# MycroftAI/mycroft-precise

Hardware: NVIDIA H100
Metric: stream-updates/s (16 kHz int16 PCM, 1024-sample chunk -> decoded confidence + trigger) (higher is better)
Workload: dtype f32

## Files before the change

### mycroft_precise_b200/csrc/api.cu

```cuda
#include <cuda_runtime.h>
#include <math.h>
#include <stdarg.h>
#include <stdint.h>
#include <stdio.h>
#include <string.h>

#include <algorithm>
#include <map>
#include <cuda_fp16.h>
#include <limits>
#include <memory>
#include <mutex>
#include <new>
#include <string>
#include <utility>
#include <vector>

#include "../../include/precise_b200.h"
#include "gru_kernels.cuh"
#include "gru_bank.cuh"
#include "gru_wide.cuh"
#include "mfcc_kernels.cuh"
#include "mfcc_fast.cuh"
#include "mfcc_ragged.cuh"
#include "mfcc_tc.cuh"
#include "mfcc_tc3.cuh"
#include "mfcc_mma.cuh"
#include "trigger.cuh"
#include "stream_state.cuh"
#include "history.cuh"
#include "corpus.cuh"
#include "corpus_pool.cuh"
#include "corpus_pairs.cuh"
#include "dataset.cuh"
#include "pool.cuh"
#include "train.cuh"
#include "noise.cuh"

#include <cub/device/device_segmented_sort.cuh>

using namespace pb;

static thread_local char g_err[512] = "";

static int fail(int code, const char* fmt, ...) {
    va_list ap;
    va_start(ap, fmt);
    vsnprintf(g_err, sizeof(g_err), fmt, ap);
    va_end(ap);
    return code;
}

#define CK(call)                                                                                  \
    do {                                                                                          \
        cudaError_t e_ = (call);                                                                  \
        if (e_ != cudaSuccess)                                                                    \
            return fail(PB_ERR_CUDA, "%s failed: %s (%s:%d)", #call, cudaGetErrorString(e_), __FILE__, __LINE__); \
    } while (0)

constexpr int N_PROFILE_SLOTS = 4;
constexpr int PROFILE_POOL = 2048;
constexpr int K2_WARP_PATH_MAX = 8192;
constexpr int64_t HOST_ZERO_COPY_MAX = 64;
constexpr int HOST_PIPE = 3;
constexpr int64_t HOST_SUB_BATCH = 16384;

struct ProfSlot {
    std::vector<cudaEvent_t> ev;
    int used = 0;
    double ms = 0.0;
    uint64_t launches = 0;
};

template <typename T>
class DevArray {
public:
    DevArray() = default;
    DevArray(DevArray&& o) noexcept : p_(o.p_), n_(o.n_) { o.p_ = nullptr; o.n_ = 0; }
    DevArray& operator=(DevArray&& o) noexcept { std::swap(p_, o.p_); std::swap(n_, o.n_); return *this; }
    DevArray(const DevArray&) = delete;
    DevArray& operator=(const DevArray&) = delete;
    ~DevArray() { if (p_) cudaFree(p_); }

    cudaError_t alloc(size_t n) {
        T* p = nullptr;
        const cudaError_t e = cudaMalloc((void**)&p, std::max<size_t>(n, 1) * sizeof(T));
        if (e != cudaSuccess) return e;
        DevArray fresh;
        fresh.p_ = p; fresh.n_ = n;
        *this = std::move(fresh);
        return cudaSuccess;
    }
    cudaError_t upload(const std::vector<T>& v) {
        DevArray fresh;
        cudaError_t e = fresh.alloc(v.size());
        if (e == cudaSuccess && !v.empty()) e = cudaMemcpy(fresh.p_, v.data(), v.size() * sizeof(T), cudaMemcpyHostToDevice);
        if (e == cudaSuccess) *this = std::move(fresh);
        return e;
    }
    T* get() const { return p_; }
    size_t size() const { return n_; }

private:
    T* p_ = nullptr;
    size_t n_ = 0;
};

struct NetWeights {
    bool small_path = false;
    GruSmallW<20, 13> w_small;
    DevArray<float> wcat, bias, wd;
    float bd = 0.f;
    DevArray<uint4> bfrag16;
    DevArray<uint4> xfrag16;
    DevArray<float> mma_bias, mma_wd;
    bool wide_ok = false;
    int wg_fp = 0, wg_hp = 0;
    DevArray<uint4> wg_b1, wg_b2; DevArray<float> wg_bias;
};

struct StreamTrig {
    double sensitivity;
    int32_t trigger_level;
    int32_t chunk_bytes;
};

struct Network {
    pb_config cfg;
    std::vector<double> cd;
    int min_out = 0, max_out = 0;
    DevArray<double> d_cd;
    DevArray<int> trig;
    int gru_mode = 0;
    std::unique_ptr<NetWeights> w;
    bool trig_set = false;
    std::vector<StreamTrig> trig_host;
    DevArray<TrigRec> trig_rec;
};

struct pb_handle {
    pb_config cfg;
    int sm_count = 132;
    int used = 0, n_bins = 0, n_out = 0, feat = 0, ring_rows = 0, row_stride = 0, tail_cap = 0, max_new = 0;
    int rel_window = 0;
    size_t k1_batch_smem = 0, k1_stream_smem = 0, k1_fast_smem = 0, k1_pipe_smem = 0, k1_ragged_smem = 0;
    bool ragged = false;
    bool force_generic = false;
    int k1_mode = 0;
    bool mma_ok = false;
    DevArray<uint2> d_mm_b1, d_mm_b2; DevArray<float2> d_mm_tw;
    DevArray<MmRec> d_mm_recs; DevArray<unsigned int> d_mm_counters;
    int mm_parity = 0;
    bool fast_ok = false;
    int npl = 0, maxc = 0, nol = 0;
    DevArray<float4> d_ptab;
    DevArray<unsigned char> d_ctab;
    DevArray<float> d_dct_t;
    bool pipe_fixed = false;
    DevArray<int4> d_pm_off; DevArray<float4> d_pm_w; DevArray<uint4> d_pm_crow; DevArray<float4> d_pm_dct;
    std::vector<double> fb;
    DevArray<float> d_wrise, d_wfall, d_dct;
    DevArray<int> d_grid;
    DevArray<float2> d_tw_stage, d_tw_post, d_tw_any;
    DevArray<long long> d_n_samples;
    DevArray<int16_t> d_tail;
    DevArray<float> d_ring;
    std::vector<Network> models;
    bool routed = false;
    std::vector<uint8_t> route_mask;
    int64_t subs[PB_MAX_MODELS] = {};
    DevArray<uint8_t> d_route;
    DevArray<int2> d_route_list;
    DevArray<unsigned> d_route_count;
// ... 719 lines not shown
                    power257[k] = (k == 0 || k == 256) ? re * re * inv : (re * re + im * im) * inv;
                }
    }
    return PB_OK;
}

PB_API int pb_debug_mma_dft_power(const int16_t* x512, double* power257) {
    if (!x512 || !power257) return fail(PB_ERR_INVALID, "null argument");
    mm_host_power(x512, power257);
    return PB_OK;
}

PB_API int pb_debug_force_generic(pb_handle* h, int on) { if (!h) return fail(PB_ERR_INVALID, "null handle"); h->force_generic = on != 0; return PB_OK; }

PB_API int pb_profile_enable(pb_handle* h, int on) { if (!h) return fail(PB_ERR_INVALID, "null handle"); h->profiling = on != 0; return PB_OK; }

PB_API int pb_profile_reset(pb_handle* h) {
    if (!h) return fail(PB_ERR_INVALID, "null handle");
    for (auto& p : h->prof) { p.used = 0; p.ms = 0; p.launches = 0; }
    return PB_OK;
}

PB_API int pb_profile_read(pb_handle* h, double ms[4], uint64_t launches[4]) {
    if (!h) return fail(PB_ERR_INVALID, "null handle");
    CK(cudaSetDevice(h->cfg.device));
    for (int s = 0; s < N_PROFILE_SLOTS; ++s) {
        ProfSlot& p = h->prof[s];
        for (int i = 0; i + 1 < p.used; i += 2) {
            CK(cudaEventSynchronize(p.ev[i + 1]));
            float t = 0; CK(cudaEventElapsedTime(&t, p.ev[i], p.ev[i + 1])); p.ms += t;
        }
        p.used = 0;
        if (ms) ms[s] = p.ms;
        if (launches) launches[s] = p.launches;
    }
    return PB_OK;
}

static MelTables mel_tables(const pb_handle* h) {
    MelTables t;
    t.w_rise = h->d_wrise.get(); t.w_fall = h->d_wfall.get(); t.grid = h->d_grid.get(); t.dct = h->d_dct.get();
    t.tw_stage = h->d_tw_stage.get(); t.tw_post = h->d_tw_post.get();
    t.n_bins = h->n_bins; t.n_filt = h->cfg.n_filt; t.n_out = h->n_out;
    t.mels_only = h->cfg.vectorizer == PB_VEC_MELS;
    t.n_fft = h->cfg.n_fft; t.tw_any = h->d_tw_any.get();
    return t;
}

static FastTables fast_tables(const pb_handle* h) {
    FastTables f;
    f.ptab = h->d_ptab.get(); f.ctab = h->d_ctab.get(); f.dct_t = h->d_dct_t.get();
    f.npl = h->npl; f.maxc = h->maxc; f.nol = h->nol;
    return f;
}

static StreamState stream_state(const pb_handle* h) {
    StreamState st;
    st.n_samples = h->d_n_samples.get(); st.tail = h->d_tail.get(); st.ring = h->d_ring.get();
    st.tail_cap = h->tail_cap; st.ring_rows = h->ring_rows; st.row_stride = h->row_stride;
    return st;
}

static int trigger_reset(long long bytes) {
    long long q = -(8 * 2048) / bytes;
    if ((-(8 * 2048)) % bytes != 0) q -= 1;
    return (int)q;
}

static DecodeParams decode_params(const Network& net) {
    const pb_config& c = net.cfg;
    DecodeParams d;
    d.cd = net.d_cd.get(); d.cd_len = (int)net.cd.size();
    d.min_out = net.min_out; d.out_range = net.max_out - net.min_out;
    d.center = c.threshold_center;
    d.hot_threshold = 1.0 - c.sensitivity;
    d.trigger_level = c.trigger_level;
    d.trigger_reset = trigger_reset(2LL * c.chunk_samples);
    d.legacy_f64 = c.decode_legacy_f64 != 0;
    return d;
}

static StreamTrig default_trig(const Network& net) {
    return StreamTrig{net.cfg.sensitivity, net.cfg.trigger_level, (int32_t)std::min<long long>(2LL * net.cfg.chunk_samples, INT32_MAX)};
}

static TrigRec trig_record(const StreamTrig& v) {
    return TrigRec{1.0 - v.sensitivity, v.trigger_level, trigger_reset(v.chunk_bytes)};
}

static void defer_trigger(TrigTick& t, int& nt, const Network& net, unsigned route_bit, K2Out& o) {
    t.conf[nt] = o.conf; t.fired[nt] = o.fired; t.count[nt] = o.count; t.trig[nt] = o.trig;
    t.rec[nt] = net.trig_rec.get(); t.route_bit[nt] = route_bit;
    ++nt;
    o.trig = nullptr; o.fired = nullptr; o.count = nullptr;
}

static int launch_trigger(const TrigTick& t, int nt, cudaStream_t s) {
    if (nt == 0 || t.n == 0) return PB_OK;
    trigger_kernel<<<dim3((unsigned)((t.n + 255) / 256), (unsigned)nt), 256, 0, s>>>(t);
    CK(cudaGetLastError());
    return PB_OK;
}

template <typename T>
static int mfcc_impl(pb_handle* h, const T* d_in, int64_t n_streams, int64_t L, float* d_out, cudaStream_t s, float scale) {
    if (!h) return fail(PB_ERR_INVALID, "null handle");
    if (n_streams < 0 || L < 0) return fail(PB_ERR_INVALID, "negative size");
    if (L == 0 && n_streams > 0) return fail(PB_ERR_INVALID, "Cannot vectorize empty audio!");
    const int64_t nf = pb_mfcc_frames(h, L), total = nf * n_streams;
    if (total == 0) return PB_OK;
    if (!d_in || !d_out) return fail(PB_ERR_INVALID, "null buffer");
    CK(cudaSetDevice(h->cfg.device));
    const bool pairs = (L % 2 == 0) && (h->cfg.hop_samples % 2 == 0) && (h->used % 2 == 0) &&
                       ((uintptr_t)d_in % (2 * sizeof(T)) == 0);
    const int64_t tiles = (total + K1_TILE - 1) / K1_TILE;
    const int grid = (int)std::min<int64_t>(tiles, (int64_t)h->sm_count * 4);
    ProfScope ps(h, 0, s);
    if (sizeof(T) == 2 && h->fast_ok && L % 8 == 0 && (uintptr_t)d_in % 16 == 0 && !h->force_generic) {
        const int64_t pairs2 = (total + 1) / 2;
        const int gridf = (int)std::min<int64_t>((pairs2 + K1F_WARPS - 1) / K1F_WARPS, (int64_t)h->sm_count * 4);
        mfcc_fast_batch_kernel<<<gridf, K1F_THREADS, h->k1_fast_smem, s>>>((const int16_t*)d_in, L, nf, total, h->cfg.hop_samples, scale,
                                                                           mel_tables(h), fast_tables(h), d_out);
    } else if (pairs)
        mfcc_batch_kernel<T, true><<<grid, K1_THREADS, h->k1_batch_smem, s>>>(d_in, L, nf, total, h->cfg.hop_samples, h->used, scale, mel_tables(h), d_out);
    else
        mfcc_batch_kernel<T, false><<<grid, K1_THREADS, h->k1_batch_smem, s>>>(d_in, L, nf, total, h->cfg.hop_samples, h->used, scale, mel_tables(h), d_out);
    CK(cudaGetLastError());
    return PB_OK;
}

PB_API int pb_mfcc(pb_handle* h, const int16_t* d_pcm, int64_t n_streams, int64_t L, float* d_out, void* stream) {
    if (!h) return fail(PB_ERR_INVALID, "null handle");
    const float inv = 1.0f / 32768.0f;
    return mfcc_impl<int16_t>(h, d_pcm, n_streams, L, d_out, (cudaStream_t)stream, inv * inv / (float)h->cfg.n_fft);
}

PB_API int pb_mfcc_f32(pb_handle* h, const float* d_audio, int64_t n_streams, int64_t L, float* d_out, void* stream) {
    if (!h) return fail(PB_ERR_INVALID, "null handle");
    return mfcc_impl<float>(h, d_audio, n_streams, L, d_out, (cudaStream_t)stream, 1.0f / (float)h->cfg.n_fft);
}

static void set_bank_slot(BankParams& P, int slot, const Network& net, const K2Out& o) {
    const NetWeights& nw = *net.w;
    BankModelW& w = P.w[slot];
    w.bfrag = nw.bfrag16.get(); w.xfrag = nw.xfrag16.get(); w.bias = nw.mma_bias.get(); w.wd = nw.mma_wd.get(); w.bd = nw.bd;
    w.act = net.cfg.activation; w.ract = net.cfg.recurrent_activation;
    P.dp[slot] = decode_params(net);
    P.o[slot] = o;
}

template <int NM, bool RING, bool KERAS_ACT>
static int launch_bank_act(const BankParams& P, const K2In& in, int64_t n, cudaStream_t s) {
    constexpr size_t smem = (size_t)NM * BANK_MODEL_SMEM + (bank_stages(NM, RING) ? BANK_STAGE_SMEM : 0);
    if constexpr (smem > 48 * 1024) CK(ensure_dyn_smem(gru_bank_kernel<NM, RING, KERAS_ACT>, smem));
    const int per_cta = (MMA_THREADS / 32) * 16;
    gru_bank_kernel<NM, RING, KERAS_ACT><<<(int)((n + per_cta - 1) / per_cta), MMA_THREADS, smem, s>>>(P, in, n);
    CK(cudaGetLastError());
    return PB_OK;
}

template <int NM, bool RING>
static int launch_bank_nm(const BankParams& P, const K2In& in, int64_t n, cudaStream_t s) {
    if constexpr (NM == 1)
        if (P.w[0].act == PB_ACT_LINEAR && P.w[0].ract == PB_RACT_HARD_SIGMOID) return launch_bank_act<1, RING, true>(P, in, n, s);
    return launch_bank_act<NM, RING, false>(P, in, n, s);
}

static int launch_gru_kernels(const Network& net, int F, const K2In& in, bool ring, int64_t n, const K2Out& o, cudaStream_t s) {
    const NetWeights& nw = *net.w;
    const pb_config& c = net.cfg;
    const DecodeParams dp = decode_params(net);
    if (nw.small_path && n <= K2_WARP_PATH_MAX && net.gru_mode == 0) {
        const int grid = (int)((n + 3) / 4);
        if (ring) gru_warp_kernel<20, 13, true><<<grid, 128, 0, s>>>(nw.w_small, in, n, dp, o);
        else gru_warp_kernel<20, 13, false><<<grid, 128, 0, s>>>(nw.w_small, in, n, dp, o);
    } else if (nw.small_path && net.gru_mode != 1) {
        BankParams P{};
        set_bank_slot(P, 0, net, o);
        return ring ? launch_bank_nm<1, true>(P, in, n, s) : launch_bank_nm<1, false>(P, in, n, s);
    } else if (nw.small_path) {
        const int per_cta = K2_SMALL_THREADS * K2_NS;
        const int grid = (int)((n + per_cta - 1) / per_cta);
        if (ring && o.route) gru_small_kernel<20, 13, true, true><<<grid, K2_SMALL_THREADS, 0, s>>>(nw.w_small, in, n, dp, o);
        else if (ring) gru_small_kernel<20, 13, true><<<grid, K2_SMALL_THREADS, 0, s>>>(nw.w_small, in, n, dp, o);
        else gru_small_kernel<20, 13, false><<<grid, K2_SMALL_THREADS, 0, s>>>(nw.w_small, in, n, dp, o);
    } else if (nw.wide_ok && net.gru_mode != 1) {
        GruWideW w;
        w.b1 = nw.wg_b1.get(); w.b2 = nw.wg_b2.get(); w.bias = nw.wg_bias.get(); w.wd = nw.wd.get(); w.bd = nw.bd;
        w.H = c.hidden; w.F = F; w.FP = nw.wg_fp; w.HP = nw.wg_hp; w.act = c.activation; w.ract = c.recurrent_activation;
        const int grid = (int)((n + WG_STREAMS - 1) / WG_STREAMS);
        const size_t smem = wg_smem(w.FP, w.HP);
        if (ring) gru_wide_kernel<true><<<grid, WG_THREADS, smem, s>>>(w, in, n, dp, o);
        else gru_wide_kernel<false><<<grid, WG_THREADS, smem, s>>>(w, in, n, dp, o);
    } else {
        GruTiledW w;
        w.wcat = nw.wcat.get(); w.bias = nw.bias.get(); w.wd = nw.wd.get(); w.bd = nw.bd;
        w.H = c.hidden; w.F_in = F; w.act = c.activation; w.ract = c.recurrent_activation;
        const size_t smem = (size_t)(w.F_in + 3 * w.H) * K2_TILE_STREAMS * sizeof(float);
        const int grid = (int)((n + K2_TILE_STREAMS - 1) / K2_TILE_STREAMS);
        if (ring) gru_tiled_kernel<true><<<grid, K2_TILE_THREADS, smem, s>>>(w, in, n, dp, o);
        else gru_tiled_kernel<false><<<grid, K2_TILE_THREADS, smem, s>>>(w, in, n, dp, o);
    }
    CK(cudaGetLastError());
    return PB_OK;
}

static int launch_gru(pb_handle* h, const Network& net, const K2In& in, bool ring, int64_t n, const K2Out& o, cudaStream_t s) {
    ProfScope ps(h, 1, s);
    return launch_gru_kernels(net, h->feat, in, ring, n, o, s);
}

PB_API int pb_predict(pb_handle* h, const float* d_inputs, int64_t n, float* d_out, float* d_logit, void* stream) {
    if (!h) return fail(PB_ERR_INVALID, "null handle");
    if (!h->models[0].w) return fail(PB_ERR_STATE, "pb_load_weights has not been called");
    if (n < 0) return fail(PB_ERR_INVALID, "negative n");
    if (n == 0) return PB_OK;
    if (!d_inputs || !d_out) return fail(PB_ERR_INVALID, "null buffer");
    CK(cudaSetDevice(h->cfg.device));
    K2In in{};
    in.inputs = d_inputs; in.row_stride = h->feat; in.T = h->cfg.n_features; in.F_base = h->n_out; in.use_delta = 0;
    K2Out o{};
    o.raw = d_out; o.logit = d_logit;
    return launch_gru(h, h->models[0], in, false, n, o, (cudaStream_t)stream);
}

PB_API int pb_decode(pb_handle* h, const float* d_raw, int64_t n, double* d_conf, void* stream) {
    if (!h) return fail(PB_ERR_INVALID, "null handle");
    if (n < 0) return fail(PB_ERR_INVALID, "negative n");
    if (n == 0) return PB_OK;
    if (!d_raw || !d_conf) return fail(PB_ERR_INVALID, "null buffer");
    CK(cudaSetDevice(h->cfg.device));
    cudaStream_t s = (cudaStream_t)stream;
    ProfScope ps(h, 2, s);
    decode_kernel<<<(int)((n + 255) / 256), 256, 0, s>>>(d_raw, n, decode_params(h->models[0]), d_conf);
    CK(cudaGetLastError());
    return PB_OK;
}

static int check_tick(pb_handle* h, const void* pcm, int64_t n) {
    if (!h) return fail(PB_ERR_INVALID, "null handle");
    if (n < 0 || n > h->cfg.max_streams) return fail(PB_ERR_INVALID, "n = %lld outside [0, max_streams = %d]", (long long)n, h->cfg.max_streams);
    if (n > 0 && !pcm) return fail(PB_ERR_INVALID, "null pcm");
    return PB_OK;
}

static int ensure_mma_tables(pb_handle* h) {
    if (h->d_mm_b1.get()) return PB_OK;
    std::vector<uint2> b1, b2;
    std::vector<float2> tw;
    mm_build_tables(b1, b2, tw);
    CK(h->d_mm_b2.upload(b2));
    CK(h->d_mm_tw.upload(tw));
    CK(h->d_mm_recs.alloc((size_t)h->cfg.max_streams * (size_t)std::max(1, h->max_new)));
    CK(h->d_mm_counters.alloc(2));
    CK(cudaMemset(h->d_mm_counters.get(), 0, 2 * sizeof(unsigned int)));
    CK(ensure_dyn_smem(mfcc_mma_kernel<false, false>, sizeof(MmSmem)));
    CK(ensure_dyn_smem(mfcc_mma_kernel<true, false>, sizeof(MmSmem)));
    CK(ensure_dyn_smem(mfcc_mma_kernel<true, true>, sizeof(MmSmem)));
    CK(h->d_mm_b1.upload(b1));
    return PB_OK;
}

static int launch_ragged_mfcc(pb_handle* h, const int16_t* d_pcm, const int64_t* d_offsets, int64_t max_len, const int32_t* d_ids,
                              int64_t n, cudaStream_t s) {
    const float inv = 1.0f / 32768.0f, scale = inv * inv / (float)h->cfg.n_fft;
    const StreamState st = stream_state(h);
    RaggedIn rg;
    rg.offsets = reinterpret_cast<const long long*>(d_offsets);
    rg.max_len = max_len;
    rg.chunk = h->cfg.chunk_samples;
    rg.sub = 6 * h->cfg.hop_samples;
    const bool fast = h->fast_ok && !h->force_generic;
    const int64_t warps_total = (int64_t)h->sm_count * 4 * K1F_WARPS;
    const int spw = (int)std::max<int64_t>(1, std::min<int64_t>(K1F_STREAMS_PER_WARP, (n + warps_total - 1) / warps_total));
    const int64_t tilesf = (n + spw - 1) / spw;
    const int gridf = (int)std::min<int64_t>((tilesf + K1F_WARPS - 1) / K1F_WARPS, (int64_t)h->sm_count * 4);
    const int grid = (int)std::min<int64_t>((n + K1_STREAMS_PER_CTA - 1) / K1_STREAMS_PER_CTA, (int64_t)h->sm_count * 4);
    ProfScope ps(h, 0, s);
    for (int64_t off = 0; off < max_len; off += rg.sub) {
        rg.round_off = off;
        if (fast)
            mfcc_ragged_stream_kernel<<<gridf, K1F_THREADS, h->k1_ragged_smem, s>>>(d_pcm, rg, d_ids, (int)n, h->cfg.hop_samples, spw, scale,
                                                                                   mel_tables(h), fast_tables(h), st);
        else
            mfcc_stream_kernel<false, true><<<grid, K1_THREADS, h->k1_stream_smem, s>>>(d_pcm, d_ids, (int)n, 0, 0, h->cfg.hop_samples, h->used,
                                                                                       scale, mel_tables(h), st, rg);
        CK(cudaGetLastError());
    }
    return PB_OK;
}

static int launch_stream_mfcc(pb_handle* h, const int16_t* d_pcm, const int32_t* d_ids, int64_t n, cudaStream_t s) {
    if (h->ragged) return launch_ragged_mfcc(h, d_pcm, nullptr, h->cfg.chunk_samples, d_ids, n, s);
    const bool pairs = (h->cfg.chunk_samples % 2 == 0) && (h->cfg.hop_samples % 2 == 0) && (h->used % 2 == 0) &&
                       ((uintptr_t)d_pcm % 4 == 0);
    const int64_t tiles = (n + K1_STREAMS_PER_CTA - 1) / K1_STREAMS_PER_CTA;
    const int grid = (int)std::min<int64_t>(tiles, (int64_t)h->sm_count * 4);
    const float inv = 1.0f / 32768.0f, scale = inv * inv / (float)h->cfg.n_fft;
    const StreamState st = stream_state(h);
    ProfScope ps(h, 0, s);
    if (h->k1_mode >= 4 && h->mma_ok && (uintptr_t)d_pcm % 16 == 0 && !h->force_generic) {
        int rc = ensure_mma_tables(h);
        if (rc != PB_OK) return rc;
        MmTables t;
        t.b1 = h->d_mm_b1.get(); t.b2 = h->d_mm_b2.get(); t.tw = h->d_mm_tw.get();
        t.pscale = inv * inv / (float)h->cfg.n_fft * 1024.f;
        const int par = h->mm_parity;
        h->mm_parity ^= 1;
        MmRec* recs = h->d_mm_recs.get();
// ... 2446 lines not shown
```

### mycroft_precise_b200/csrc/gru_bank.cuh

```cuda
#pragma once
#include <cuda_fp16.h>

#include "gru_kernels.cuh"

namespace pb {

__device__ __forceinline__ void mma_f16_k16(float (&d)[4], const uint32_t (&a)[4], uint32_t b0, uint32_t b1) {
    asm volatile("mma.sync.aligned.m16n8k16.row.col.f32.f16.f16.f32 {%0,%1,%2,%3}, {%4,%5,%6,%7}, {%8,%9}, {%0,%1,%2,%3};"
                 : "+f"(d[0]), "+f"(d[1]), "+f"(d[2]), "+f"(d[3])
                 : "r"(a[0]), "r"(a[1]), "r"(a[2]), "r"(a[3]), "r"(b0), "r"(b1));
}
__device__ __forceinline__ void mma_f16_k8(float (&d)[4], uint32_t a0, uint32_t a1, uint32_t b0) {
    asm volatile("mma.sync.aligned.m16n8k8.row.col.f32.f16.f16.f32 {%0,%1,%2,%3}, {%4,%5}, {%6}, {%0,%1,%2,%3};"
                 : "+f"(d[0]), "+f"(d[1]), "+f"(d[2]), "+f"(d[3])
                 : "r"(a0), "r"(a1), "r"(b0));
}
__device__ __forceinline__ uint32_t pack_f16x2_sat(float x, float y) {
    uint32_t r;
    asm("cvt.rn.satfinite.f16x2.f32 %0, %1, %2;" : "=r"(r) : "f"(y), "f"(x));
    return r;
}
__device__ __forceinline__ void split_f16(float x, float y, uint32_t& hi, uint32_t& lo) {
    hi = pack_f16x2_sat(x, y);
    const float2 f = __half22float2(*reinterpret_cast<const __half2*>(&hi));
// ... 105 lines not shown
            idx[hf] = p.x;
            sid[hf] = p.y;
        } else if (RING && ok[hf]) {
            sid[hf] = in.ids ? in.ids[idx[hf]] : (int)idx[hf];
        }
        if (RING && ok[hf]) {
            if (!STAGE) {
                const long long ns = in.n_samples[sid[hf]];
                rc[hf].init(in, sid[hf], ns >= in.window ? (ns - in.window) / in.hop + 1 : 0);
            }
        }
    }
    float* stage = reinterpret_cast<float*>(bank_smem + NM * BANK_MODEL_SMEM) + warp * 2 * BANK_STAGE_BUF;
    const int cs = lane >> 1;
    const bool cok = STAGE && base + cs < n;
    RingCursor cur;
    cur.stride = 0;
    if (cok) {
        const int csid = list != nullptr ? list[base + cs].y : in.ids ? in.ids[base + cs] : (int)(base + cs);
        const long long ns = in.n_samples[csid];
        cur.init(in, csid, ns >= in.window ? (ns - in.window) / in.hop + 1 : 0);
    }
    if (STAGE) {
        bank_stage(stage, cur, cok, cs, 0, in.T, in.ring, lane);
        cp_async_commit();
        bank_stage(stage + BANK_STAGE_BUF, cur, cok, cs, BANK_STAGE_STEPS, in.T, in.ring, lane);
        cp_async_commit();
    }
    int chunk = 0, cr = 0;
    float hreg[NM][3][4];
#pragma unroll
    for (int m = 0; m < NM; ++m)
#pragma unroll
        for (int nt = 0; nt < 3; ++nt)
#pragma unroll
            for (int e = 0; e < 4; ++e) hreg[m][nt][e] = 0.f;

#pragma unroll 1
    for (int step = 0; step < in.T; ++step) {
        float xv[2][4];
        if (STAGE) {
            if (cr == 0) {
                cp_async_wait<1>();
                __syncwarp();
            }
            const float* xs = stage + (chunk & 1) * BANK_STAGE_BUF + cr * 16 * BANK_STAGE_ROW;
#pragma unroll
            for (int hf = 0; hf < 2; ++hf) {
                const float* row = xs + (g + 8 * hf) * BANK_STAGE_ROW;
                const float2 lo = *reinterpret_cast<const float2*>(row + 2 * t), hi = *reinterpret_cast<const float2*>(row + 2 * t + 8);
                xv[hf][0] = 2 * t < F ? lo.x : 0.f;
                xv[hf][1] = 2 * t + 1 < F ? lo.y : 0.f;
                xv[hf][2] = 2 * t + 8 < F ? hi.x : 0.f;
                xv[hf][3] = 2 * t + 9 < F ? hi.y : 0.f;
            }
            if (cr + 1 == BANK_STAGE_STEPS) {
                __syncwarp();
                bank_stage(stage + (chunk & 1) * BANK_STAGE_BUF, cur, cok, cs, (chunk + 2) * BANK_STAGE_STEPS, in.T, in.ring, lane);
                cp_async_commit();
                cr = 0;
                ++chunk;
            } else {
                ++cr;
            }
        } else {
#pragma unroll
            for (int hf = 0; hf < 2; ++hf) {
                const float* row = nullptr;
                if (ok[hf]) row = RING ? rc[hf].next(step) : input_row(in, idx[hf], step);
                xv[hf][0] = (row != nullptr && 2 * t < F) ? __ldg(row + 2 * t) : 0.f;
                xv[hf][1] = (row != nullptr && 2 * t + 1 < F) ? __ldg(row + 2 * t + 1) : 0.f;
                xv[hf][2] = (row != nullptr && 2 * t + 8 < F) ? __ldg(row + 2 * t + 8) : 0.f;
                xv[hf][3] = (row != nullptr && 2 * t + 9 < F) ? __ldg(row + 2 * t + 9) : 0.f;
            }
        }
        uint32_t xh[4], xl[4];
        split_f16(xv[0][0], xv[0][1], xh[0], xl[0]);
        split_f16(xv[1][0], xv[1][1], xh[1], xl[1]);
        split_f16(xv[0][2], xv[0][3], xh[2], xl[2]);
        split_f16(xv[1][2], xv[1][3], xh[3], xl[3]);
#pragma unroll
        for (int m = 0; m < NM; ++m) {
            const uint4* sB = reinterpret_cast<const uint4*>(bank_smem + (ws + m) * BANK_MODEL_SMEM);
            const uint4* sX = sB + 2 * MMA_NT * 32;
            const float* sBias = reinterpret_cast<const float*>(sB + BANK_FRAG_U4);
            const int ra = P.w[m0 + m].ract, ac = P.w[m0 + m].act;
            float acc[MMA_NT][4];
#pragma unroll
            for (int nt = 0; nt < MMA_NT; ++nt) {
                const float b0 = sBias[8 * nt + 2 * t], b1 = sBias[8 * nt + 2 * t + 1];
                acc[nt][0] = b0; acc[nt][1] = b1; acc[nt][2] = b0; acc[nt][3] = b1;
            }
#pragma unroll
            for (int ng = 0; ng < MMA_NT; ng += 3) {
                uint4 w[3];
#pragma unroll
                for (int q = 0; q < 3; ++q) w[q] = sX[(ng + q) * 32 + lane];
#pragma unroll
                for (int q = 0; q < 3; ++q) mma_f16_k16(acc[ng + q], xl, w[q].x, w[q].y);
#pragma unroll
                for (int q = 0; q < 3; ++q) mma_f16_k16(acc[ng + q], xh, w[q].z, w[q].w);
#pragma unroll
                for (int q = 0; q < 3; ++q) mma_f16_k16(acc[ng + q], xh, w[q].x, w[q].y);
            }
            {
                uint32_t ah[4], al[4], ch[2], cl[2];
                frag_f16(hreg[m], ah, al, ch, cl);
                mma3_f16(acc, 0, ah, al, ch, cl, sB, lane);
                mma3_f16(acc, 3, ah, al, ch, cl, sB, lane);
            }
            {
                float rh[3][4];
#pragma unroll
                for (int nt = 0; nt < 3; ++nt)
#pragma unroll
                    for (int e = 0; e < 4; ++e) {
                        const float r = KERAS_ACT ? hard_sigmoid(acc[3 + nt][e]) : apply_ract(acc[3 + nt][e], ra);
                        rh[nt][e] = __fmul_rn(r, hreg[m][nt][e]);
                    }
                uint32_t ah[4], al[4], ch[2], cl[2];
                frag_f16(rh, ah, al, ch, cl);
                mma3_f16(acc, 6, ah, al, ch, cl, sB, lane);
            }
#pragma unroll
            for (int nt = 0; nt < 3; ++nt)
#pragma unroll
                for (int e = 0; e < 4; ++e) {
                    const float z = KERAS_ACT ? hard_sigmoid(acc[nt][e]) : apply_ract(acc[nt][e], ra);
                    const float a = KERAS_ACT ? acc[6 + nt][e] : apply_act(acc[6 + nt][e], ac);
                    hreg[m][nt][e] = __fmaf_rn(z, hreg[m][nt][e], __fmul_rn(__fsub_rn(1.f, z), a));
                }
        }
    }
    if (STAGE) cp_async_wait<0>();
#pragma unroll
    for (int m = 0; m < NM; ++m) {
        const float* sWd = reinterpret_cast<const float*>(bank_smem + (ws + m) * BANK_MODEL_SMEM + BANK_FRAG_U4 * 16) + 72;
#pragma unroll
        for (int hf = 0; hf < 2; ++hf) {
            float part = 0.f;
#pragma unroll
            for (int nt = 0; nt < 3; ++nt) {
                part = fmaf(hreg[m][nt][2 * hf], sWd[8 * nt + 2 * t], part);
                part = fmaf(hreg[m][nt][2 * hf + 1], sWd[8 * nt + 2 * t + 1], part);
            }
            part += __shfl_xor_sync(0xffffffffu, part, 1);
            part += __shfl_xor_sync(0xffffffffu, part, 2);
            epilogue(part + P.w[m0 + m].bd, t == 0 && ok[hf], idx[hf], sid[hf], P.dp[m0 + m], P.o[m0 + m]);
        }
    }
}

template <int NM, bool RING, bool KERAS_ACT>
__global__ void __launch_bounds__(MMA_THREADS, NM == 1 ? 4 : 1)
gru_bank_kernel(const __grid_constant__ BankParams P, K2In in, long long n) {
    bank_scan<NM, RING, KERAS_ACT>(P, 0, nullptr, blockIdx.x, in, n);
}

struct BankRoute {
    const int2* list[BANK_MAX_MODELS];
    const unsigned* count[BANK_MAX_MODELS];
    int tile0[BANK_MAX_MODELS + 1];
    int nm;
};

struct RouteOut {
    float* raw;
    double* conf;
    uint8_t* fired;
    int M;
    int2* lists;
    long long list_stride;
    unsigned* count;
    unsigned listed;
};

__global__ void __launch_bounds__(256) route_kernel(const uint8_t* route, const int* ids, long long n, RouteOut r) {
    const long long i = (long long)blockIdx.x * blockDim.x + threadIdx.x;
    const bool ok = i < n;
    const int sid = ok ? (ids ? ids[i] : (int)i) : 0;
    const unsigned mask = ok ? route[sid] : 0u;
    const int lane = threadIdx.x & 31;
    for (int m = 0; m < r.M; ++m) {
        const unsigned bit = 1u << m;
        const long long o = (long long)m * n + i;
        if (ok && !(mask & bit)) {
            if (r.raw) r.raw[o] = __int_as_float(0x7fc00000);
            r.conf[o] = __longlong_as_double(0x7ff8000000000000LL);
            if (r.fired) r.fired[o] = 0;
        }
        if (r.lists != nullptr && (r.listed & bit)) {
            const bool sub = ok && (mask & bit);
            const unsigned b = __ballot_sync(0xffffffffu, sub);
            if (b == 0) continue;
            unsigned at = 0;
            if (lane == 0) at = atomicAdd(r.count + m, (unsigned)__popc(b));
            at = __shfl_sync(0xffffffffu, at, 0);
            if (sub) r.lists[m * r.list_stride + at + __popc(b & ((1u << lane) - 1u))] = make_int2((int)i, sid);
        }
    }
}

template <bool KERAS_ACT>
__global__ void __launch_bounds__(MMA_THREADS, 4)
gru_bank_routed_kernel(const __grid_constant__ BankParams P, const __grid_constant__ BankRoute R, K2In in) {
    int k = 0;
    while (k + 1 < R.nm && (int)blockIdx.x >= R.tile0[k + 1]) ++k;
    const long long tile = (long long)blockIdx.x - R.tile0[k];
    const long long n = *R.count[k];
    if (tile * (MMA_THREADS / 32) * 16 >= n) return;
    bank_scan<1, true, KERAS_ACT>(P, k, R.list[k], tile, in, n);
}

}
```

Measured before the change: 305.2 million.

## Replace per-warp mma.sync GRU scan with Hopper wgmma kernel for single-model bank

Adds a new GRU scan kernel for the single-model bank path. It stores the split-fp16 weight tiles in shared memory in the wgmma core-matrix layout and issues warpgroup-level wgmma.mma_async (m64n24/48/72) instead of per-warp m16n8k16 mma.sync. The aim is fewer instructions per recurrent step and operand reuse across the warpgroup, at the cost of async fence/commit/wait overhead on every step. The multi-model bank kernel's launch bounds are relaxed to one block per SM, since single-model launches now go to the new kernel.

```diff
diff --git a/mycroft_precise_b200/csrc/api.cu b/mycroft_precise_b200/csrc/api.cu
--- a/mycroft_precise_b200/csrc/api.cu
+++ b/mycroft_precise_b200/csrc/api.cu
@@ -19,6 +19,7 @@
 #include "../../include/precise_b200.h"
 #include "gru_kernels.cuh"
 #include "gru_bank.cuh"
+#include "gru_wg.cuh"
 #include "gru_wide.cuh"
 #include "mfcc_kernels.cuh"
 #include "mfcc_fast.cuh"
@@ -1044,9 +1045,15 @@
 template <int NM, bool RING, bool KERAS_ACT>
 static int launch_bank_act(const BankParams& P, const K2In& in, int64_t n, cudaStream_t s) {
     constexpr size_t smem = (size_t)NM * BANK_MODEL_SMEM + (bank_stages(NM, RING) ? BANK_STAGE_SMEM : 0);
-    if constexpr (smem > 48 * 1024) CK(ensure_dyn_smem(gru_bank_kernel<NM, RING, KERAS_ACT>, smem));
     const int per_cta = (MMA_THREADS / 32) * 16;
-    gru_bank_kernel<NM, RING, KERAS_ACT><<<(int)((n + per_cta - 1) / per_cta), MMA_THREADS, smem, s>>>(P, in, n);
+    const int grid = (int)((n + per_cta - 1) / per_cta);
+    if constexpr (NM == 1) {
+        if constexpr (smem > 48 * 1024) CK(ensure_dyn_smem(gru_wg_kernel<RING, KERAS_ACT>, smem));
+        gru_wg_kernel<RING, KERAS_ACT><<<grid, MMA_THREADS, smem, s>>>(P, in, n);
+    } else {
+        if constexpr (smem > 48 * 1024) CK(ensure_dyn_smem(gru_bank_kernel<NM, RING, KERAS_ACT>, smem));
+        gru_bank_kernel<NM, RING, KERAS_ACT><<<grid, MMA_THREADS, smem, s>>>(P, in, n);
+    }
     CK(cudaGetLastError());
     return PB_OK;
 }
diff --git a/mycroft_precise_b200/csrc/gru_bank.cuh b/mycroft_precise_b200/csrc/gru_bank.cuh
--- a/mycroft_precise_b200/csrc/gru_bank.cuh
+++ b/mycroft_precise_b200/csrc/gru_bank.cuh
@@ -281,7 +281,7 @@
 }
 
 template <int NM, bool RING, bool KERAS_ACT>
-__global__ void __launch_bounds__(MMA_THREADS, NM == 1 ? 4 : 1)
+__global__ void __launch_bounds__(MMA_THREADS, 1)
 gru_bank_kernel(const __grid_constant__ BankParams P, K2In in, long long n) {
     bank_scan<NM, RING, KERAS_ACT>(P, 0, nullptr, blockIdx.x, in, n);
 }
diff --git a/mycroft_precise_b200/csrc/gru_wg.cuh b/mycroft_precise_b200/csrc/gru_wg.cuh
--- /dev/null
+++ b/mycroft_precise_b200/csrc/gru_wg.cuh
@@ -0,0 +1,235 @@
+#pragma once
+#include <stdint.h>
+
+#include "gru_bank.cuh"
+
+namespace pb {
+
+constexpr int WG_TILE_BYTES = 72 * 16 * 2;
+__host__ __device__ constexpr int wg_b_offset(int k, int n) { return (n >> 3) * 256 + (k >> 3) * 128 + (n & 7) * 16 + (k & 7) * 2; }
+
+__device__ __forceinline__ uint64_t wg_desc(const void* p) {
+    const uint32_t a = (uint32_t)__cvta_generic_to_shared(p);
+    return (uint64_t)((a & 0x3ffff) >> 4) | ((uint64_t)(128 >> 4) << 16) | ((uint64_t)(256 >> 4) << 32);
+}
+
+__device__ __forceinline__ void wg_fence() { asm volatile("wgmma.fence.sync.aligned;" ::: "memory"); }
+__device__ __forceinline__ void wg_commit() { asm volatile("wgmma.commit_group.sync.aligned;" ::: "memory"); }
+template <int N>
+__device__ __forceinline__ void wg_wait() { asm volatile("wgmma.wait_group.sync.aligned %0;" :: "n"(N) : "memory"); }
+__device__ __forceinline__ void wg_fence_smem() { asm volatile("fence.proxy.async.shared::cta;" ::: "memory"); }
+template <int N>
+__device__ __forceinline__ void wg_fence_regs(float* d) {
+#pragma unroll
+    for (int i = 0; i < N; ++i) asm volatile("" : "+f"(d[i]) :: "memory");
+}
+
+__device__ __forceinline__ void wgmma_n24(float* d, const uint32_t (&a)[4], uint64_t desc) {
+    asm volatile("{\n.reg .pred p;\nsetp.ne.b32 p, %17, 0;\n"
+                 "wgmma.mma_async.sync.aligned.m64n24k16.f32.f16.f16 "
+                 "{%0,%1,%2,%3,%4,%5,%6,%7,%8,%9,%10,%11}, {%12,%13,%14,%15}, %16, p, 1, 1, 0;\n}\n"
+                 : "+f"(d[0]), "+f"(d[1]), "+f"(d[2]), "+f"(d[3]), "+f"(d[4]), "+f"(d[5]), "+f"(d[6]), "+f"(d[7]),
+                   "+f"(d[8]), "+f"(d[9]), "+f"(d[10]), "+f"(d[11])
+                 : "r"(a[0]), "r"(a[1]), "r"(a[2]), "r"(a[3]), "l"(desc), "r"(1));
+}
+__device__ __forceinline__ void wgmma_n48(float* d, const uint32_t (&a)[4], uint64_t desc) {
+    asm volatile("{\n.reg .pred p;\nsetp.ne.b32 p, %29, 0;\n"
+                 "wgmma.mma_async.sync.aligned.m64n48k16.f32.f16.f16 "
+                 "{%0,%1,%2,%3,%4,%5,%6,%7,%8,%9,%10,%11,%12,%13,%14,%15,%16,%17,%18,%19,%20,%21,%22,%23}, "
+                 "{%24,%25,%26,%27}, %28, p, 1, 1, 0;\n}\n"
+                 : "+f"(d[0]), "+f"(d[1]), "+f"(d[2]), "+f"(d[3]), "+f"(d[4]), "+f"(d[5]), "+f"(d[6]), "+f"(d[7]),
+                   "+f"(d[8]), "+f"(d[9]), "+f"(d[10]), "+f"(d[11]), "+f"(d[12]), "+f"(d[13]), "+f"(d[14]), "+f"(d[15]),
+                   "+f"(d[16]), "+f"(d[17]), "+f"(d[18]), "+f"(d[19]), "+f"(d[20]), "+f"(d[21]), "+f"(d[22]), "+f"(d[23])
+                 : "r"(a[0]), "r"(a[1]), "r"(a[2]), "r"(a[3]), "l"(desc), "r"(1));
+}
+__device__ __forceinline__ void wgmma_n72(float* d, const uint32_t (&a)[4], uint64_t desc) {
+    asm volatile("{\n.reg .pred p;\nsetp.ne.b32 p, %41, 0;\n"
+                 "wgmma.mma_async.sync.aligned.m64n72k16.f32.f16.f16 "
+                 "{%0,%1,%2,%3,%4,%5,%6,%7,%8,%9,%10,%11,%12,%13,%14,%15,%16,%17,%18,%19,%20,%21,%22,%23,"
+                 "%24,%25,%26,%27,%28,%29,%30,%31,%32,%33,%34,%35}, {%36,%37,%38,%39}, %40, p, 1, 1, 0;\n}\n"
+                 : "+f"(d[0]), "+f"(d[1]), "+f"(d[2]), "+f"(d[3]), "+f"(d[4]), "+f"(d[5]), "+f"(d[6]), "+f"(d[7]),
+                   "+f"(d[8]), "+f"(d[9]), "+f"(d[10]), "+f"(d[11]), "+f"(d[12]), "+f"(d[13]), "+f"(d[14]), "+f"(d[15]),
+                   "+f"(d[16]), "+f"(d[17]), "+f"(d[18]), "+f"(d[19]), "+f"(d[20]), "+f"(d[21]), "+f"(d[22]), "+f"(d[23]),
+                   "+f"(d[24]), "+f"(d[25]), "+f"(d[26]), "+f"(d[27]), "+f"(d[28]), "+f"(d[29]), "+f"(d[30]), "+f"(d[31]),
+                   "+f"(d[32]), "+f"(d[33]), "+f"(d[34]), "+f"(d[35])
+                 : "r"(a[0]), "r"(a[1]), "r"(a[2]), "r"(a[3]), "l"(desc), "r"(1));
+}
+
+template <bool RING, bool KERAS_ACT>
+__global__ void __launch_bounds__(MMA_THREADS, 4)
+gru_wg_kernel(const __grid_constant__ BankParams P, K2In in, long long n) {
+    extern __shared__ __align__(16) unsigned char bank_smem[];
+    const BankModelW& w = P.w[0];
+    unsigned char* sW = bank_smem;
+    float* sb = reinterpret_cast<float*>(bank_smem + BANK_FRAG_U4 * 16);
+    for (int e = threadIdx.x; e < 3 * MMA_NT * 32; e += blockDim.x) {
+        const int kt = e / (MMA_NT * 32), nt = (e / 32) % MMA_NT, lane = e & 31, col = 8 * nt + (lane >> 2), k = 2 * (lane & 3);
+        const uint4 f = kt < 2 ? __ldg(w.bfrag + e) : __ldg(w.xfrag + e - 2 * MMA_NT * 32);
+        unsigned char* hi = sW + (kt == 2 ? 0 : 2 + 2 * kt) * WG_TILE_BYTES;
+        unsigned char* lo = hi + WG_TILE_BYTES;
+        *reinterpret_cast<uint32_t*>(hi + wg_b_offset(k, col)) = f.x;
+        *reinterpret_cast<uint32_t*>(hi + wg_b_offset(k + 8, col)) = f.y;
+        *reinterpret_cast<uint32_t*>(lo + wg_b_offset(k, col)) = f.z;
+        *reinterpret_cast<uint32_t*>(lo + wg_b_offset(k + 8, col)) = f.w;
+    }
+    for (int e = threadIdx.x; e < 72; e += blockDim.x) sb[e] = __ldg(w.bias + e);
+    for (int e = threadIdx.x; e < 24; e += blockDim.x) sb[72 + e] = __ldg(w.wd + e);
+    wg_fence_smem();
+    __syncthreads();
+    const int lane = threadIdx.x & 31, warp = threadIdx.x >> 5, g = lane >> 2, t = lane & 3;
+    const long long base = ((long long)blockIdx.x * (MMA_THREADS / 32) + warp) * 16;
+    constexpr bool STAGE = RING;
+    const int F = in.F_base;
+    long long idx[2];
+    int sid[2];
+    bool ok[2];
+#pragma unroll
+    for (int hf = 0; hf < 2; ++hf) {
+        idx[hf] = base + g + 8 * hf;
+        ok[hf] = idx[hf] < n;
+        sid[hf] = RING && ok[hf] ? (in.ids ? in.ids[idx[hf]] : (int)idx[hf]) : 0;
+    }
+    float* stage = reinterpret_cast<float*>(bank_smem + BANK_MODEL_SMEM) + warp * 2 * BANK_STAGE_BUF;
+    const int cs = lane >> 1;
+    const bool cok = STAGE && base + cs < n;
+    RingCursor cur;
+    cur.stride = 0;
+    if (cok) {
+        const int csid = in.ids ? in.ids[base + cs] : (int)(base + cs);
+        const long long ns = in.n_samples[csid];
+        cur.init(in, csid, ns >= in.window ? (ns - in.window) / in.hop + 1 : 0);
+    }
+    if (STAGE) {
+        bank_stage(stage, cur, cok, cs, 0, in.T, in.ring, lane);
+        cp_async_commit();
+        bank_stage(stage + BANK_STAGE_BUF, cur, cok, cs, BANK_STAGE_STEPS, in.T, in.ring, lane);
+        cp_async_commit();
+    }
+    const uint64_t dXh = wg_desc(sW), dXl = wg_desc(sW + WG_TILE_BYTES), dU0h = wg_desc(sW + 2 * WG_TILE_BYTES),
+                   dU0l = wg_desc(sW + 3 * WG_TILE_BYTES), dU1h = wg_desc(sW + 4 * WG_TILE_BYTES), dU1l = wg_desc(sW + 5 * WG_TILE_BYTES);
+    constexpr uint64_t C6 = (6 * 256) >> 4;
+    const int ra = w.ract, ac = w.act;
+    int chunk = 0, cr = 0;
+    float h[3][4] = {};
+
+#pragma unroll 1
+    for (int step = 0; step < in.T; ++step) {
+        float xv[2][4];
+        if (STAGE) {
+            if (cr == 0) {
+                cp_async_wait<1>();
+                __syncwarp();
+            }
+            const float* xs = stage + (chunk & 1) * BANK_STAGE_BUF + cr * 16 * BANK_STAGE_ROW;
+#pragma unroll
+            for (int hf = 0; hf < 2; ++hf) {
+                const float* row = xs + (g + 8 * hf) * BANK_STAGE_ROW;
+                const float2 lo = *reinterpret_cast<const float2*>(row + 2 * t), hi = *reinterpret_cast<const float2*>(row + 2 * t + 8);
+                xv[hf][0] = 2 * t < F ? lo.x : 0.f;
+                xv[hf][1] = 2 * t + 1 < F ? lo.y : 0.f;
+                xv[hf][2] = 2 * t + 8 < F ? hi.x : 0.f;
+                xv[hf][3] = 2 * t + 9 < F ? hi.y : 0.f;
+            }
+            if (cr + 1 == BANK_STAGE_STEPS) {
+                __syncwarp();
+                bank_stage(stage + (chunk & 1) * BANK_STAGE_BUF, cur, cok, cs, (chunk + 2) * BANK_STAGE_STEPS, in.T, in.ring, lane);
+                cp_async_commit();
+                cr = 0;
+                ++chunk;
+            } else {
+                ++cr;
+            }
+        } else {
+#pragma unroll
+            for (int hf = 0; hf < 2; ++hf) {
+                const float* row = ok[hf] ? input_row(in, idx[hf], step) : nullptr;
+                xv[hf][0] = (row != nullptr && 2 * t < F) ? __ldg(row + 2 * t) : 0.f;
+                xv[hf][1] = (row != nullptr && 2 * t + 1 < F) ? __ldg(row + 2 * t + 1) : 0.f;
+                xv[hf][2] = (row != nullptr && 2 * t + 8 < F) ? __ldg(row + 2 * t + 8) : 0.f;
+                xv[hf][3] = (row != nullptr && 2 * t + 9 < F) ? __ldg(row + 2 * t + 9) : 0.f;
+            }
+        }
+        uint32_t xh[4], xl[4];
+        split_f16(xv[0][0], xv[0][1], xh[0], xl[0]);
+        split_f16(xv[1][0], xv[1][1], xh[1], xl[1]);
+        split_f16(xv[0][2], xv[0][3], xh[2], xl[2]);
+        split_f16(xv[1][2], xv[1][3], xh[3], xl[3]);
+        float acc[36];
+#pragma unroll
+        for (int nt = 0; nt < MMA_NT; ++nt) {
+            const float b0 = sb[8 * nt + 2 * t], b1 = sb[8 * nt + 2 * t + 1];
+            acc[4 * nt] = b0; acc[4 * nt + 1] = b1; acc[4 * nt + 2] = b0; acc[4 * nt + 3] = b1;
+        }
+        uint32_t ah[4], al[4], ch[4] = {0u, 0u, 0u, 0u}, cl[4] = {0u, 0u, 0u, 0u};
+        {
+            uint32_t c2h[2], c2l[2];
+            frag_f16(h, ah, al, c2h, c2l);
+            ch[0] = c2h[0]; ch[1] = c2h[1]; cl[0] = c2l[0]; cl[1] = c2l[1];
+        }
+        wg_fence_regs<36>(acc);
+        wg_fence();
+        wgmma_n48(acc, xl, dXh);
+        wgmma_n24(acc + 24, xl, dXh + C6);
+        wgmma_n48(acc, xh, dXl);
+        wgmma_n24(acc + 24, xh, dXl + C6);
+        wgmma_n48(acc, xh, dXh);
+        wgmma_n24(acc + 24, xh, dXh + C6);
+        wgmma_n48(acc, al, dU0h);
+        wgmma_n48(acc, cl, dU1h);
+        wgmma_n48(acc, ah, dU0l);
+        wgmma_n48(acc, ch, dU1l);
+        wgmma_n48(acc, ah, dU0h);
+        wgmma_n48(acc, ch, dU1h);
+        wg_commit();
+        wg_wait<0>();
+        wg_fence_regs<36>(acc);
+        {
+            float rh[3][4];
+#pragma unroll
+            for (int nt = 0; nt < 3; ++nt)
+#pragma unroll
+                for (int e = 0; e < 4; ++e) {
+                    const float r = KERAS_ACT ? hard_sigmoid(acc[4 * (3 + nt) + e]) : apply_ract(acc[4 * (3 + nt) + e], ra);
+                    rh[nt][e] = __fmul_rn(r, h[nt][e]);
+                }
+            uint32_t c2h[2], c2l[2];
+            frag_f16(rh, ah, al, c2h, c2l);
+            ch[0] = c2h[0]; ch[1] = c2h[1]; cl[0] = c2l[0]; cl[1] = c2l[1];
+        }
+        wg_fence_regs<12>(acc + 24);
+        wg_fence();
+        wgmma_n24(acc + 24, al, dU0h + C6);
+        wgmma_n24(acc + 24, cl, dU1h + C6);
+        wgmma_n24(acc + 24, ah, dU0l + C6);
+        wgmma_n24(acc + 24, ch, dU1l + C6);
+        wgmma_n24(acc + 24, ah, dU0h + C6);
+        wgmma_n24(acc + 24, ch, dU1h + C6);
+        wg_commit();
+        wg_wait<0>();
+        wg_fence_regs<12>(acc + 24);
+#pragma unroll
+        for (int nt = 0; nt < 3; ++nt)
+#pragma unroll
+            for (int e = 0; e < 4; ++e) {
+                const float z = KERAS_ACT ? hard_sigmoid(acc[4 * nt + e]) : apply_ract(acc[4 * nt + e], ra);
+                const float a = KERAS_ACT ? acc[4 * (6 + nt) + e] : apply_act(acc[4 * (6 + nt) + e], ac);
+                h[nt][e] = __fmaf_rn(z, h[nt][e], __fmul_rn(__fsub_rn(1.f, z), a));
+            }
+    }
+    if (STAGE) cp_async_wait<0>();
+    const float* sWd = sb + 72;
+#pragma unroll
+    for (int hf = 0; hf < 2; ++hf) {
+        float part = 0.f;
+#pragma unroll
+        for (int nt = 0; nt < 3; ++nt) {
+            part = fmaf(h[nt][2 * hf], sWd[8 * nt + 2 * t], part);
+            part = fmaf(h[nt][2 * hf + 1], sWd[8 * nt + 2 * t + 1], part);
+        }
+        part += __shfl_xor_sync(0xffffffffu, part, 1);
+        part += __shfl_xor_sync(0xffffffffu, part, 2);
+        epilogue(part + w.bd, t == 0 && ok[hf], idx[hf], sid[hf], P.dp[0], P.o[0]);
+    }
+}
+
+}
```

Result: faster. 339.0 million (median of 6 runs) (+11.1%).
